# peter-nebe/stair-step-detector

Measured on AMD Instinct MI355X. Metric: point-cloud frames/sec (1024×768 pts) at 1/2/4/8 GPUs; step height/corner max-abs err, higher is better.
Workload: dtype f64; 1 GPU; BASELINE configs[2]: batch of 1024 synthetic 1024x768 frames (3-step staircases, randomised rise/tread/yaw/noise) resident in HBM, streamed through the whole per-frame path; per GPU; width=1024, height=768, input=float3, risers=False, batches_in_flight=3, parallelism=frame-sharded x1, no collective

## Files before the change

include/ssd_testhooks.h:

```cpp
#ifndef SSD_TESTHOOKS_H_
#define SSD_TESTHOOKS_H_

#include "ssd_hip.h"

#ifdef __cplusplus
extern "C" {
#endif

double ssd_test_hypot_host(double a, double b);
int ssd_test_hypot_device(int device, const double *a, const double *b, double *out, int n);
int ssd_test_sort_host(const double *dist, int n, int32_t *perm);
int ssd_test_sort_device(int device, const double *dist, int n, int32_t *perm);
int ssd_test_quad_device(int device, const double quad[8], const double *pts_xy, int n, uint8_t *inside, int *err);
int ssd_test_quad_host(const double quad[8], const double *pts_xy, int n, uint8_t *inside, int *err);
int ssd_test_quad_edges_host(const double quad[8], const double range[6], const double a[9], const double b[3], const float *pts_xyz, int n,
                             float consts[15], int8_t *cls, double *world_xy, uint8_t *in_range_xy, int *err);
int ssd_test_quad_edges_device(int device, const double *quads, int n, const double range_xy[4], float *out);
int ssd_test_best_line_host(const int32_t *pts_xy, int n, int form, int32_t line[3]);
int ssd_test_closing_host(const uint8_t *img, int width, int height, int x0, int x_step, int y_from, int band_rows, uint8_t *closed_out,
                          int32_t *first, int32_t *last, int n_cols);
int ssd_test_grid_boxes_device(int device, const double quad[8], double x_min, double y_min, double box_x, double box_y,
                               const int32_t *boxes, int n, uint8_t *inside, int *usable);
long long ssd_test_frame_state(ssd_handle *h, int frame, void *out, size_t cap, long long layout[8]);
int ssd_test_empty_quadrilateral(ssd_handle *h, int frame, int surface);
int ssd_test_single_pass(ssd_handle *h, int mode, int sabotage);
int ssd_test_plane_pool(ssd_handle *h, int planes);
int ssd_test_single_pass_stats(ssd_handle *h, int frames, int scan_planes, long long counts[4]);
int ssd_test_single_pass_frame(ssd_handle *h, int frame, uint8_t *plane_of_bin, int info[3]);
int ssd_test_single_pass_sample(ssd_handle *h, int frame, uint32_t *sample);
int ssd_test_predict_table_host(const uint32_t *sample, int n_bins, int min_height, int sabotage, uint8_t *plane_of_bin);
int ssd_test_prexy_host(const double range[6], const double a[9], const double b[3], float out[14]);
int ssd_test_prez_host(const double range[6], const double a[9], const double b[3], double height_interval, int width, int height, float out[16]);
int ssd_test_record_offset(ssd_handle *h, size_t offset_bytes);
unsigned long long ssd_test_record_realloc(ssd_handle *h);
unsigned long long ssd_test_record_realloc_sized(ssd_handle *h, size_t extra_bytes, size_t offset_bytes);
int ssd_test_record_release(void);
int ssd_test_ground_image(ssd_handle *h, int frame, uint8_t *out);
int ssd_test_line_host(const double pq[4], double abc_d[3], int32_t abc_i[3]);
int ssd_test_intersect_host(const double l[3], const double o[3], double xy[2]);

int ssd_test_stream_read(int device, const void *d_ptr, size_t bytes, int reps, void *stream, float *ms_avg);

const char *ssd_testhooks_last_error(void);

#ifdef __cplusplus
}
#endif

#endif
```

stair-step-detector_amd/__init__.py:

```python
import ctypes as C
import math
import os

import numpy as np

_HERE = os.path.dirname(os.path.abspath(__file__))
LIB_PATH = os.environ.get("SSD_HIP_LIB") or os.path.join(_HERE, "lib", "libssd_hip.so")

MAX_BINS = 128
MAX_PLATEAUS = 32
MAX_STEP_IMAGES = 16
MAX_PLANES = 24
POOL_PLANES_PER_FRAME = 10


def plane_pool_size(frames, points_per_frame):
    per = 16 if points_per_frame < 600000 else POOL_PLANES_PER_FRAME
    return max(frames * per + 2 * MAX_PLANES, min(frames, 8) * MAX_PLANES)
MAX_STEPS = MAX_STEP_IMAGES + 1
MAX_SCANS = 128
MAX_EDGE_PTS = 256
LINE_CAP = 4096

ST_THROW, ST_OOB_PIXEL, ST_ASSERT, ST_OVERFLOW = 1, 2, 4, 8
# ... 155 lines not shown
                ("seed", C.c_uint64)]


EXPORTS = [
    "ssd_default_config", "ssd_calibration_from_points", "ssd_calibration_identity", "ssd_calibration_load",
    "ssd_create", "ssd_destroy", "ssd_last_error", "ssd_workspace_bytes",
    "ssd_process_host", "ssd_enqueue", "ssd_fetch", "ssd_enqueue_stages",
    "ssd_set_intrinsics", "ssd_process_depth_host", "ssd_enqueue_depth", "ssd_deproject_host",
    "ssd_fetch_back", "ssd_stream_wait", "ssd_batches_in_flight", "ssd_set_risers", "ssd_set_single_pass", "ssd_fetch_risers", "ssd_set_timing", "ssd_get_stage_times", "ssd_get_stage_times_back", "ssd_get_predict_time_back", "ssd_serialize",
    "ssd_set_debug", "ssd_get_debug", "ssd_get_debug_image",
    "ssd_device_count", "ssd_device_alloc", "ssd_device_free", "ssd_device_upload", "ssd_device_download",
    "ssd_device_sync", "ssd_host_alloc", "ssd_host_free", "ssd_device_info_get", "ssd_bind_thread_to_device",
    "ssd_pipeline_create", "ssd_pipeline_destroy", "ssd_pipeline_submit", "ssd_pipeline_submit_after", "ssd_pipeline_next", "ssd_pipeline_pending", "ssd_pipeline_set_timing", "ssd_pipeline_stage_times",
    "ssd_pipeline_last_error",
    "ssd_enqueue_labels", "ssd_enqueue_depth_labels", "ssd_process_host_labels", "ssd_process_depth_host_labels", "ssd_get_labels_time_back",
    "ssd_set_cameras", "ssd_camera_count", "ssd_enqueue_cameras", "ssd_process_host_cameras",
    "ssd_calibration_from_plane", "ssd_ground_moments_host", "ssd_ground_fit_solve", "ssd_enqueue_ground_fit", "ssd_fetch_ground_fit",
    "ssd_process_host_ground_fit",
    "ssd_enqueue_surface_moments", "ssd_enqueue_depth_surface_moments", "ssd_get_surface_moments_time_back", "ssd_surface_moments_host",
    "ssd_surface_fit_solve", "ssd_process_host_surfaces",
    "ssd_enqueue_cameras_surface_moments", "ssd_process_host_cameras_surfaces", "ssd_camera_drift_fold",
    "ssd_set_riser_moments", "ssd_fetch_riser_moments", "ssd_riser_fit_solve", "ssd_process_host_riser_fits",
    "ssd_process_host_cameras_riser_fits",
    "ssd_surface_gates_from_moments", "ssd_surface_refit_moments_host", "ssd_enqueue_surface_refit", "ssd_fetch_surface_refit",
    "ssd_get_surface_refit_time", "ssd_process_host_surfaces_refit",
    "ssd_enqueue_cameras_surface_refit", "ssd_process_host_cameras_surfaces_refit", "ssd_camera_ground_gates",
]
SOURCE_EXPORTS = [
    "ssd_synth_generate_host", "ssd_synth_generate_device", "ssd_synth_depth_host", "ssd_synth_depth_device",
    "ssd_synth_scene_to_camera", "ssd_source_default_scene", "ssd_source_write_calibration", "ssd_source_last_error",
]
HOOK_EXPORTS = [
    "ssd_test_hypot_host", "ssd_test_hypot_device", "ssd_test_frame_state", "ssd_test_ground_image", "ssd_test_line_host", "ssd_test_intersect_host", "ssd_test_quad_device", "ssd_test_quad_host", "ssd_test_closing_host", "ssd_test_best_line_host", "ssd_test_grid_boxes_device", "ssd_test_sort_host",
    "ssd_test_sort_device", "ssd_test_stream_read", "ssd_test_empty_quadrilateral", "ssd_test_single_pass", "ssd_test_plane_pool", "ssd_test_single_pass_stats", "ssd_test_single_pass_frame", "ssd_test_single_pass_sample", "ssd_test_predict_table_host", "ssd_test_prexy_host", "ssd_test_prez_host", "ssd_test_quad_edges_host", "ssd_test_quad_edges_device", "ssd_test_record_offset", "ssd_test_record_realloc", "ssd_test_record_realloc_sized", "ssd_test_record_release", "ssd_testhooks_last_error",
]
SOURCE_LIB_PATH = os.path.join(os.path.dirname(LIB_PATH), "libssd_source.so")
HOOKS_LIB_PATH = os.path.join(os.path.dirname(LIB_PATH), "libssd_testhooks.so")

_lib = None
_source_lib = None
_hooks_lib = None


def lib():
    global _lib
    if _lib is not None:
        return _lib
    if not os.path.exists(LIB_PATH):
        raise SsdError("%s is missing: build it with `python -c 'import __graft_entry__ as g; g.build()'` "
                       "(or make -C stair-step-detector_amd/csrc); there is no CPU fallback" % LIB_PATH)
    L = C.CDLL(LIB_PATH)
    vp, i32, sz = C.c_void_p, C.c_int, C.c_size_t
    L.ssd_last_error.restype = C.c_char_p
    L.ssd_workspace_bytes.restype = sz
    L.ssd_workspace_bytes.argtypes = [vp]
    L.ssd_default_config.argtypes = [C.POINTER(Config), i32, i32]
    L.ssd_calibration_from_points.argtypes = [C.POINTER(C.c_double), C.POINTER(C.c_double), C.POINTER(Calibration)]
    L.ssd_calibration_identity.argtypes = [C.POINTER(Calibration)]
    L.ssd_calibration_load.argtypes = [C.c_char_p, C.c_char_p, C.POINTER(Calibration), C.POINTER(C.c_int),
                                       C.POINTER(C.c_double), C.POINTER(C.c_double)]
    L.ssd_create.argtypes = [C.POINTER(Config), C.POINTER(Calibration), i32, C.POINTER(vp)]
    L.ssd_destroy.argtypes = [vp]
    L.ssd_process_host.argtypes = [vp, vp, i32, C.POINTER(FrameResult)]
    L.ssd_enqueue.argtypes = [vp, vp, sz, i32, vp]
    L.ssd_enqueue_stages.argtypes = [vp, vp, sz, i32, vp, i32]
    L.ssd_fetch.argtypes = [vp, C.POINTER(FrameResult), i32, vp]
    L.ssd_set_intrinsics.argtypes = [vp, C.POINTER(Intrinsics)]
# ... 100 lines not shown
    _source_lib = L
    return L


def hooks_lib():
    global _hooks_lib
    if _hooks_lib is not None:
        return _hooks_lib
    if not os.path.exists(HOOKS_LIB_PATH):
        raise SsdError("%s is missing: build it with make -C stair-step-detector_amd/csrc" % HOOKS_LIB_PATH)
    lib()
    L = C.CDLL(HOOKS_LIB_PATH)
    vp, i32 = C.c_void_p, C.c_int
    L.ssd_testhooks_last_error.restype = C.c_char_p
    L.ssd_test_hypot_host.restype = C.c_double
    L.ssd_test_hypot_host.argtypes = [C.c_double, C.c_double]
    L.ssd_test_hypot_device.argtypes = [i32, vp, vp, vp, i32]
    L.ssd_test_closing_host.argtypes = [vp, i32, i32, i32, i32, i32, i32, vp, vp, vp, i32]
    L.ssd_test_closing_host.restype = i32
    L.ssd_test_best_line_host.argtypes = [vp, i32, i32, vp]
    L.ssd_test_best_line_host.restype = i32
    L.ssd_test_quad_host.argtypes = [vp, vp, i32, vp, vp]
    L.ssd_test_quad_host.restype = i32
    L.ssd_test_frame_state.argtypes = [vp, i32, vp, C.c_size_t, vp]
    L.ssd_test_frame_state.restype = C.c_longlong
    L.ssd_test_ground_image.argtypes = [vp, i32, vp]
    L.ssd_test_empty_quadrilateral.argtypes = [vp, i32, i32]
    L.ssd_test_single_pass.argtypes = [vp, i32, i32]
    L.ssd_test_plane_pool.argtypes = [vp, i32]
    L.ssd_test_single_pass_stats.argtypes = [vp, i32, i32, vp]
    L.ssd_test_single_pass_frame.argtypes = [vp, i32, vp, vp]
    L.ssd_test_single_pass_sample.argtypes = [vp, i32, vp]
    L.ssd_test_predict_table_host.argtypes = [vp, i32, i32, i32, vp]
    L.ssd_test_prexy_host.argtypes = [vp, vp, vp, vp]
    L.ssd_test_prez_host.argtypes = [vp, vp, vp, C.c_double, i32, i32, vp]
    L.ssd_test_quad_edges_host.argtypes = [vp, vp, vp, vp, vp, i32, vp, vp, vp, vp, vp]
    L.ssd_test_quad_edges_host.restype = i32
    L.ssd_test_quad_edges_device.argtypes = [i32, vp, i32, vp, vp]
    L.ssd_test_quad_edges_device.restype = i32
    L.ssd_test_record_offset.argtypes = [vp, C.c_size_t]
    L.ssd_test_record_realloc.argtypes = [vp]
    L.ssd_test_record_realloc.restype = C.c_ulonglong
    L.ssd_test_record_realloc_sized.argtypes = [vp, C.c_size_t, C.c_size_t]
    L.ssd_test_record_realloc_sized.restype = C.c_ulonglong
    L.ssd_test_line_host.argtypes = [vp, vp, vp]
    L.ssd_test_intersect_host.argtypes = [vp, vp, vp]
    L.ssd_test_sort_host.argtypes = [vp, i32, vp]
    L.ssd_test_sort_device.argtypes = [i32, vp, i32, vp]
    L.ssd_test_quad_device.argtypes = [i32, vp, vp, i32, vp, C.POINTER(C.c_int)]
    L.ssd_test_grid_boxes_device.argtypes = [i32, vp, C.c_double, C.c_double, C.c_double, C.c_double, vp, i32, vp, C.POINTER(C.c_int)]
    L.ssd_test_stream_read.argtypes = [i32, vp, C.c_size_t, i32, vp, C.POINTER(C.c_float)]
    _hooks_lib = L
    return L


def _check(rc, which="hip"):
    if rc < 0:
        msg = {"hip": lambda: lib().ssd_last_error(), "source": lambda: source_lib().ssd_source_last_error(),
               "hooks": lambda: hooks_lib().ssd_testhooks_last_error()}[which]().decode()
        raise SsdError("libssd_%s error %d: %s" % (which, rc, msg))
    return rc


def predict_table_host(sample, n_bins, min_height, sabotage=0):
    a = np.ascontiguousarray(sample, dtype=np.uint32)
    assert a.size == MAX_BINS
    out = np.zeros(MAX_BINS, dtype=np.uint8)
    n = _check(hooks_lib().ssd_test_predict_table_host(a.ctypes.data_as(C.c_void_p), n_bins, min_height, sabotage, out.ctypes.data_as(C.c_void_p)), "hooks")
    return out, n


def device_info(device):
    info = DeviceInfo()
    _check(lib().ssd_device_info_get(device, C.byref(info)))
    return {"pci_bus_id": info.pci_bus_id.decode(), "uuid": info.uuid.decode(), "numa_node": int(info.numa_node),
            "n_local_cpus": int(info.n_local_cpus), "cpu_list": info.cpu_list.decode()}


def bind_thread_to_device(device):
    n = lib().ssd_bind_thread_to_device(device)
    if n < 0:
        _check(n)
    return n


def device_count():
    return lib().ssd_device_count()


def default_config(width, height, max_frames_per_batch=64, max_step_plateaus=MAX_STEP_IMAGES, batches_in_flight=0):
    cfg = Config()
    _check(lib().ssd_default_config(C.byref(cfg), width, height))
    cfg.max_frames_per_batch = max_frames_per_batch
    cfg.max_step_plateaus = max_step_plateaus
    cfg.batches_in_flight = batches_in_flight
    return cfg


def _as_camera(prior, intr=None):
    if isinstance(prior, Camera):
        return prior
    if isinstance(prior, (tuple, list)):
# ... 926 lines not shown
```

stair-step-detector_amd/csrc/ssd_kernels.hip:

```cpp
#ifndef SSD_CAMERAS_TU
#define SSD_ENTRY(bounds, kernel, block) __global__ bounds void kernel
#define SSD_BYVAL(T) T
#else
#define SSD_ENTRY(bounds, kernel, block) __device__ __forceinline__ void block
#define SSD_BYVAL(T) const T &
#undef SSD_PHASE_TIMING
#undef SSD_COUNT
#endif
#include "ssd_device.h"
#include "ssd_moments.h"
#include "ssd_math.h"
#include "ssd_quadtest.h"
#include "ssd_closing.h"
#include "ssd_bestline.h"
#include "ssd_sort.h"

namespace ssd
{

#include "ssd_phase.h"

#ifdef SSD_CHECKED
__device__ __noinline__ void ssd_chk_report(int site, unsigned long long idx, unsigned long long limit)
{
  printf("SSD_CHECK site %d index %llu limit %llu block (%u, %u) thread %u\n", site, idx, limit, blockIdx.x, blockIdx.y, threadIdx.x);
}
__device__ __forceinline__ bool ssd_chk(int site, unsigned long long idx, unsigned long long limit)
{
  if(idx < limit)
    return true;
  ssd_chk_report(site, idx, limit);
  return false;
}
#define SSD_CHK(site, idx, limit) ssd_chk((site), static_cast<unsigned long long>(idx), static_cast<unsigned long long>(limit))
#else
#define SSD_CHK(site, idx, limit) (true)
#endif

#ifdef SSD_COUNT
__device__ unsigned long long ssd_k1_counters[8];
#define SSD_CNT(i, n) do { if(threadIdx.x % 64 == 0) atomicAdd(&ssd_k1_counters[i], static_cast<unsigned long long>(n)); } while(0)
#define SSD_CNT_LANES(i, pred) do { const unsigned long long cnt_m = __ballot(pred); if(threadIdx.x % 64 == 0 && cnt_m) atomicAdd(&ssd_k1_counters[i], static_cast<unsigned long long>(__popcll(cnt_m))); } while(0)
#else
#define SSD_CNT(i, n) do { } while(0)
#define SSD_CNT_LANES(i, pred) do { } while(0)
#endif


// ... 1105 lines not shown
__global__ __launch_bounds__(kThreads, SSD_K1S_WAVES) void k_hist_planes(const float *__restrict__ xyz, size_t strideFloats, PointParams P, PreXY Q, PixelParams X,
                                                   FrameState *__restrict__ st, uint2 *__restrict__ tileMasks,
                                                   unsigned long long *__restrict__ planeImg,
                                                   size_t tileMaskStride, int chunkPoints, DepthSrc D)
{
  __shared__ HistLds L;
  __shared__ SpecLds SL;
#ifdef SSD_K1_ROTATE
  const int chunkIdx = static_cast<int>((blockIdx.y + blockIdx.x * SSD_K1_ROTATE) % gridDim.y);
  const int frameIdx = static_cast<int>(blockIdx.x);
#elif defined(SSD_K1_ORDER)
  const int nF = static_cast<int>(gridDim.x), nC = static_cast<int>(gridDim.y);
  const int lin = static_cast<int>(blockIdx.y) * nF + static_cast<int>(blockIdx.x);
  int frameIdx, chunkIdx;
  if(SSD_K1_ORDER == 2 && (nF & 7) == 0)
  {
    const int xcd = lin & 7, i = lin >> 3;
    frameIdx = xcd + 8 * (i / nC);
    chunkIdx = i % nC;
  }
  else
  {
    frameIdx = lin / nC;
    chunkIdx = lin % nC;
  }
#else
  const int chunkIdx = static_cast<int>(blockIdx.y);
  const int frameIdx = static_cast<int>(blockIdx.x);
#endif
  hist_block<SRC, true, STRIPS, CHECKS>(L, SL, xyz, strideFloats, P, Q, X, st, tileMasks, planeImg, tileMaskStride, chunkPoints, D, frameIdx, chunkIdx);
}
#endif

template<int SRC>
SSD_ENTRY(__launch_bounds__(kThreads), k_predict, predict_block)(const float *__restrict__ xyz, size_t strideFloats, SSD_BYVAL(PointParams) P,
                                                      FrameState *__restrict__ st, SSD_BYVAL(DepthSrc) D, int minHeight, int sabotage, int *__restrict__ fallback, int poolPlanes)
{
  __shared__ unsigned int sh[kMaxBins + 2];
  __shared__ unsigned int shc[kMaxBins * kHistCopies];
  __shared__ int sLast;
  const int frame = blockIdx.x, part = blockIdx.y, nParts = gridDim.y, tid = threadIdx.x;
  const float *base = SRC == kSrcDepth16
    ? reinterpret_cast<const float *>(reinterpret_cast<const unsigned short *>(xyz) + static_cast<size_t>(frame) * strideFloats)
    : xyz + static_cast<size_t>(frame) * strideFloats;
  if(tid < kMaxBins + 2)
    sh[tid] = 0u;
  for(int i = tid; i < kMaxBins * kHistCopies; i += kThreads)
    shc[i] = 0u;
  __syncthreads();
  unsigned int *mine = shc + (tid & (kHistCopies - 1));
#ifndef SSD_K0_RUN
#define SSD_K0_RUN 16
#endif
  constexpr int kRun = SSD_K0_RUN, kLanesPerRun = kRun / kPts;
  const int nRuns = (P.nPoints + kRun - 1) / kRun;
  const int nGroups = (nRuns + kSpecSample - 1) / kSpecSample;
  for(int g = part * (kThreads / kLanesPerRun) + tid / kLanesPerRun; g < nGroups; g += nParts * (kThreads / kLanesPerRun))
  {
    const int run = g * kSpecSample + ((g * 5) & (kSpecSample - 1));
    F3 v[kPts];
    load_points<SRC>(base, run * kRun + kPts * (tid % kLanesPerRun), P.nPoints, v, D);
#pragma unroll
    for(int j = 0; j < kPts; j++)
    {
      double wx, wy, wz;
      if(world_point_flat(P, v[j], wx, wy, wz))
        atomicAdd(mine + height_bin(P, wz) * kHistCopies, 1u);
    }
  }
  __syncthreads();
  FrameState &fs = st[frame];
  if(tid < P.nBins)
  {
    unsigned int c = 0;
#pragma unroll
    for(int k = 0; k < kHistCopies; k++)
      c += shc[tid * kHistCopies + ((k + tid) & (kHistCopies - 1))];
    if(c)
    {
      const unsigned int before = atomicAdd(&fs.predHist[tid], c);
      asm volatile("" :: "v"(before));
    }
  }
  __syncthreads();
#if defined(__HIP_DEVICE_COMPILE__) && !defined(__gfx950__)
#error "k_predict's hand-over between blocks is written for gfx950 (see the comment above)"
#endif
  if(tid == 0)
    sLast = atomicAdd(&fs.predDone, 1u) == static_cast<unsigned int>(nParts - 1) ? 1 : 0;
  __syncthreads();
  if(!sLast)
    return;
  const unsigned int mineCount = tid < P.nBins ? atomicExch(&fs.predHist[tid], 0u) : 0u;
  __syncthreads();
  if(tid < kMaxBins)
  {
    sh[1 + tid] = mineCount;
    fs.predSample[tid] = mineCount;
  }
  if(tid == 0)
// ... 59 lines not shown
      if(base + total > poolPlanes)
        base = -1;
    }
    sBase = base;
  }
  __syncthreads();
  const bool fits = sBase >= 0;
  if(tid < kMaxBins)
  {
    const unsigned long long upTo = tid < 64 ? (2ull << tid) - 1ull : ~0ull;
    const int n = tid < 64 ? __popcll(sStart[0] & upTo) : __popcll(sStart[0]) + __popcll(sStart[1] & ((2ull << (tid - 64)) - 1ull));
    fs.specPlane[tid] = (want && fits) ? static_cast<unsigned char>(n - 1) : static_cast<unsigned char>(0xff);
  }
  if(tid < kMaxPlanes)
  {
    fs.planeYMin[tid] = 0x7fffffff; fs.planeYMax[tid] = -1;
    fs.planeXMin[tid] = 0x7fffffff; fs.planeXMax[tid] = -1;
    fs.planeTotZ[tid] = 0;
    fs.planeOob[tid] = 0u;
    fs.planeUsed[tid] = 0;
  }
  if(tid == 0)
  {
    fs.nPlanes = fits ? total : 0;
    fs.planeBase = fits ? sBase : 0;
    fs.predDone = 0u;
    if(frame == 0)
    {
      fallback[0] = 0;
      fallback[1] = 0;
    }
  }
}


SSD_ENTRY(__launch_bounds__(64), k_peaks, peaks_block)(SSD_BYVAL(Params) P, FrameState *__restrict__ st, int nframes, DebugFrame *__restrict__ dbg, int spec, int *__restrict__ fallback)
{
  __shared__ unsigned char sImgPlane[kMaxStepImages][2];
  __shared__ unsigned int sCovered;
  __shared__ unsigned int hist[kMaxBins + 1];
  __shared__ unsigned char lut[kMaxBins];
  __shared__ int plPeak[kMaxPlateaus], plLo[kMaxPlateaus], plHi[kMaxPlateaus], plEffLo[kMaxPlateaus], plEffHi[kMaxPlateaus], plN[kMaxPlateaus];
  __shared__ int dbgPeaks[kMaxPlateaus];
  __shared__ int sNPl, sNPeaks, sOverflow, sGround, sFirstStep, sNImg;

  const int frame = blockIdx.x, lane = threadIdx.x;
  if(frame >= nframes)
    return;
  FrameState &fs = st[frame];
  const int nb = P.nBins;

  unsigned int total = 0;
  for(int b = lane; b <= kMaxBins; b += 64)
  {
    const unsigned int v = b < nb ? fs.histAcc[b] : 0u;
    hist[b] = v;
    total += v;
    if(b < kMaxBins)
    {
      lut[b] = 0xff;
      fs.hist[b] = v;
      if(b < nb)
        fs.histAcc[b] = 0u;
    }
  }
#pragma unroll
// ... 2686 lines not shown
static inline void with_src(const DepthSrc *depth, bool aligned, F f)
{
  if(depth)
    f(std::integral_constant<int, kSrcDepth16>{}, *depth);
  else if(aligned)
    f(std::integral_constant<int, kSrcF3Aligned>{}, DepthSrc{});
  else
    f(std::integral_constant<int, kSrcF3>{}, DepthSrc{});
}
template<typename F>
static inline void with_bool(bool b, F f)
{
  if(b)
    f(std::true_type{});
  else
    f(std::false_type{});
}
}

#ifndef SSD_CAMERAS_TU
namespace ssd
{



void launch_predict(const float *xyz, size_t strideFloats, const Params &P, FrameState *st, int nframes, const DepthSrc *depth,
                    int *fallback, int poolPlanes, int sabotage, hipStream_t s, const CameraSel *cams)
{
  if(cams)
    return launch_predict_cams(xyz, strideFloats, P, st, nframes, depth, fallback, poolPlanes, sabotage, s, *cams);
  dim3 pgrid(nframes, kPredictParts);
  with_src(depth, aligned16(xyz, strideFloats, P.nPoints), [&](auto src, const DepthSrc &D)
  {
    hipLaunchKernelGGL(k_predict<decltype(src)::value>, pgrid, dim3(kThreads), 0, s, xyz, strideFloats, P.pt, st, D, P.minHeight, sabotage, fallback, poolPlanes);
  });
}
void launch_hist(const float *xyz, size_t strideFloats, const Params &P, FrameState *st, uint2 *tileMasks, size_t tileMaskStride,
                 int nframes, int chunkPoints, const DepthSrc *depth, unsigned long long *planeImg, hipStream_t s, const CameraSel *cams)
{
  if(cams)
    return launch_hist_cams(xyz, strideFloats, P, st, tileMasks, tileMaskStride, nframes, chunkPoints, depth, planeImg, s, *cams);
  dim3 grid(nframes, chunks_for(P.nPoints, chunkPoints));
  const bool strips = planeImg && kTile % P.W != 0;
  with_src(depth, aligned16(xyz, strideFloats, P.nPoints), [&](auto src, const DepthSrc &D)
  {
    with_bool(needs_checks(P), [&](auto checks)
    {
      constexpr int SRC = decltype(src)::value;
      constexpr bool CHECKS = decltype(checks)::value;
      if(planeImg)
        with_bool(strips, [&](auto sorted)
        {
          hipLaunchKernelGGL((k_hist_planes<SRC, decltype(sorted)::value, CHECKS>), grid, dim3(kThreads), 0, s, xyz, strideFloats, P.pt, P.pre, P.px, st, tileMasks, planeImg, tileMaskStride, chunkPoints, D);
        });
      else
        hipLaunchKernelGGL((k_hist<SRC, CHECKS>), grid, dim3(kThreads), 0, s, xyz, strideFloats, P.pt, P.pre, st, tileMasks, tileMaskStride, chunkPoints, D);
    });
  });
}
void launch_peaks(const Params &P, FrameState *st, int nframes, DebugFrame *dbg, int *fallback, hipStream_t s, const CameraSel *cams)
{
  if(cams)
    return launch_peaks_cams(P, st, nframes, dbg, fallback, s, *cams);
  hipLaunchKernelGGL(k_peaks, dim3(nframes), dim3(64), 0, s, P, st, nframes, dbg, fallback ? 1 : 0, fallback);
}
void launch_raster(const float *xyz, size_t strideFloats, const Params &P, FrameState *st, unsigned long long *stepImg,
                   const uint2 *tileMasks, size_t tileMaskStride, int nframes, int chunkPoints, const DepthSrc *depth, const int *fallback, hipStream_t s, const CameraSel *cams)
// ... 123 lines not shown
```

stair-step-detector_amd/csrc/ssd_kernels_cams.hip:

```cpp
#define SSD_CAMERAS_TU
#include "ssd_kernels.hip"

namespace ssd
{

template<int SRC, bool CHECKS>
__global__ __launch_bounds__(kThreads, 6) void k_hist_cams(const float *__restrict__ xyz, size_t strideFloats, const CameraRec *__restrict__ cams,
                                                        const int *__restrict__ camOf, FrameState *__restrict__ st, uint2 *__restrict__ tileMasks,
                                                        size_t tileMaskStride, int chunkPoints)
{
  __shared__ HistLds L;
  NoSpecLds none;
  const CameraRec &C = camera_of(cams, camOf, blockIdx.x);
  const PointParams P = C.P.pt;
  const PreXY Q = C.P.pre;
  const DepthSrc D = C.D;
  hist_block<SRC, false, false, CHECKS>(L, none, xyz, strideFloats, P, Q, PixelParams{}, st, tileMasks, nullptr, tileMaskStride, chunkPoints, D, blockIdx.x, blockIdx.y);
}

template<int SRC, bool STRIPS, bool CHECKS>
__global__ __launch_bounds__(kThreads, SSD_K1S_WAVES) void k_hist_planes_cams(const float *__restrict__ xyz, size_t strideFloats, const CameraRec *__restrict__ cams,
                                                   const int *__restrict__ camOf, FrameState *__restrict__ st, uint2 *__restrict__ tileMasks,
                                                   unsigned long long *__restrict__ planeImg, size_t tileMaskStride, int chunkPoints)
{
  __shared__ HistLds L;
  __shared__ SpecLds SL;
  const CameraRec &C = camera_of(cams, camOf, blockIdx.x);
  const PointParams P = C.P.pt;
  const PreXY Q = C.P.pre;
  const PixelParams X = C.P.px;
  const DepthSrc D = C.D;
  hist_block<SRC, true, STRIPS, CHECKS>(L, SL, xyz, strideFloats, P, Q, X, st, tileMasks, planeImg, tileMaskStride, chunkPoints, D, blockIdx.x, blockIdx.y);
}

template<int SRC>
__global__ __launch_bounds__(kThreads) void k_predict_cams(const float *__restrict__ xyz, size_t strideFloats, const CameraRec *__restrict__ cams,
                                                           const int *__restrict__ camOf, FrameState *__restrict__ st, int sabotage, int *__restrict__ fallback, int poolPlanes)
{
  const CameraRec &C = camera_of(cams, camOf, blockIdx.x);
  const PointParams P = C.P.pt;
  const DepthSrc D = C.D;
  predict_block<SRC>(xyz, strideFloats, P, st, D, C.P.minHeight, sabotage, fallback, poolPlanes);
}

__global__ __launch_bounds__(64) void k_peaks_cams(const CameraRec *__restrict__ cams, const int *__restrict__ camOf, FrameState *__restrict__ st, int nframes,
                                                   DebugFrame *__restrict__ dbg, int spec, int *__restrict__ fallback)
{
  if(static_cast<int>(blockIdx.x) >= nframes)
    return;
  peaks_block(camera_of(cams, camOf, blockIdx.x).P, st, nframes, dbg, spec, fallback);
}

template<int SRC, bool LIST>
__global__ __launch_bounds__(kThreads, LIST ? 5 : SSD_K2_WAVES) void k_raster_cams(const float *__restrict__ xyz, size_t strideFloats, const CameraRec *__restrict__ cams,
                                                        const int *__restrict__ camOf, FrameState *__restrict__ st,
                                                        unsigned long long *__restrict__ stepImg,
                                                        const uint2 *__restrict__ tileMasks, size_t tileMaskStride, int chunkPoints,
                                                        const int *__restrict__ fallback)
{
  __shared__ RasterLds L;
  if constexpr(LIST)
  {
    const int n = fallback[0];
    for(int e = blockIdx.x; e < n; e += gridDim.x)
    {
      const int frame = fallback[kFallbackList + e];
      const CameraRec &C = camera_of(cams, camOf, frame);
      const PointParams P = C.P.pt;
      const PixelParams X = C.P.px;
      const DepthSrc D = C.D;
      raster_block<SRC>(L, xyz, strideFloats, P, X, st, stepImg, tileMasks, tileMaskStride, chunkPoints, D, frame, blockIdx.y);
      __syncthreads();
    }
  }
  else
// ... 85 lines not shown
  const PointParams P = C.P.pt;
  const DepthSrc D = C.D;
  risers_block<SRC>(xyz, strideFloats, P, C.P.riserTol, st, tileMasks, tileMaskStride, chunkPoints, C.P.px.cellCols, D);
}

template<int SRC>
__global__ __launch_bounds__(kThreads) void k_riser_moments_cams(const float *__restrict__ xyz, size_t strideFloats, const CameraRec *__restrict__ cams,
                                                                 const int *__restrict__ camOf, FrameState *__restrict__ st, const uint2 *__restrict__ tileMasks,
                                                                 size_t tileMaskStride, int chunkPoints, ssd_frame_moments *__restrict__ out)
{
  const CameraRec &C = camera_of(cams, camOf, blockIdx.x);
  const PointParams P = C.P.pt;
  const DepthSrc D = C.D;
  riser_moments_block<SRC>(xyz, strideFloats, P, C.P.riserTol, st, tileMasks, tileMaskStride, chunkPoints, C.P.px.cellCols, D, out);
}

__global__ void k_riser_results_cams(const CameraRec *__restrict__ cams, const int *__restrict__ camOf, const FrameState *__restrict__ st,
                                     ssd_frame_risers *__restrict__ out, int nframes)
{
  const int frame = blockIdx.x * blockDim.x + threadIdx.x;
  if(frame >= nframes)
    return;
  riser_results_block(cams[camOf[frame]].P, st, out, nframes);
}



void launch_predict_cams(const float *xyz, size_t strideFloats, const Params &P, FrameState *st, int nframes, const DepthSrc *depth,
                         int *fallback, int poolPlanes, int sabotage, hipStream_t s, const CameraSel &cams)
{
  dim3 pgrid(nframes, kPredictParts);
  with_src(depth, aligned16(xyz, strideFloats, P.nPoints), [&](auto src, const DepthSrc &)
  {
    hipLaunchKernelGGL(k_predict_cams<decltype(src)::value>, pgrid, dim3(kThreads), 0, s, xyz, strideFloats, cams.table, cams.index, st, sabotage, fallback, poolPlanes);
  });
}
void launch_hist_cams(const float *xyz, size_t strideFloats, const Params &P, FrameState *st, uint2 *tileMasks, size_t tileMaskStride,
                      int nframes, int chunkPoints, const DepthSrc *depth, unsigned long long *planeImg, hipStream_t s, const CameraSel &cams)
{
  dim3 grid(nframes, chunks_for(P.nPoints, chunkPoints));
  const bool strips = planeImg && kTile % P.W != 0;
  with_src(depth, aligned16(xyz, strideFloats, P.nPoints), [&](auto src, const DepthSrc &)
  {
    with_bool(cams.checks, [&](auto checks)
    {
      constexpr int SRC = decltype(src)::value;
      constexpr bool CHECKS = decltype(checks)::value;
      if(planeImg)
        with_bool(strips, [&](auto sorted)
        {
          hipLaunchKernelGGL((k_hist_planes_cams<SRC, decltype(sorted)::value, CHECKS>), grid, dim3(kThreads), 0, s, xyz, strideFloats, cams.table, cams.index, st, tileMasks, planeImg, tileMaskStride, chunkPoints);
        });
      else
        hipLaunchKernelGGL((k_hist_cams<SRC, CHECKS>), grid, dim3(kThreads), 0, s, xyz, strideFloats, cams.table, cams.index, st, tileMasks, tileMaskStride, chunkPoints);
    });
  });
}
void launch_peaks_cams(const Params &, FrameState *st, int nframes, DebugFrame *dbg, int *fallback, hipStream_t s, const CameraSel &cams)
{
  hipLaunchKernelGGL(k_peaks_cams, dim3(nframes), dim3(64), 0, s, cams.table, cams.index, st, nframes, dbg, fallback ? 1 : 0, fallback);
}
void launch_raster_cams(const float *xyz, size_t strideFloats, const Params &P, FrameState *st, unsigned long long *stepImg,
                        const uint2 *tileMasks, size_t tileMaskStride, int nframes, int chunkPoints, const DepthSrc *depth, const int *fallback, hipStream_t s,
                        const CameraSel &cams)
{
  dim3 grid(fallback ? (nframes + 3) / 4 : nframes, chunks_for(P.nPoints, chunkPoints));
  with_src(depth, aligned16(xyz, strideFloats, P.nPoints), [&](auto src, const DepthSrc &)
// ... 91 lines not shown
```

stair-step-detector_amd/csrc/ssd_predict.h:

```cpp
#ifndef SSD_PREDICT_H_
#define SSD_PREDICT_H_

#include "ssd_device.h"

namespace ssd
{

__host__ __device__ inline bool predict_candidate(const unsigned int *sample, int nBins, int minHeight, int b)
{
  if(b < (minHeight > 1 ? minHeight : 1) || b >= nBins - 1)
    return false;
  const unsigned int c = sample[b], l = sample[b - 1], r = sample[b + 1];
  return c > l && c >= r && c * static_cast<unsigned int>(kSpecSample) >= 1200u && (l + r) * 2u < 3u * c + 16u;
}

__host__ __device__ inline int predict_table(const unsigned int *sample, int nBins, int minHeight, int sabotage, unsigned char *plane)
{
  unsigned char code[kMaxBins];
  for(int b = 0; b < kMaxBins; b++)
  {
    code[b] = 0;
    plane[b] = 0xff;
  }
  if(sabotage == 2)
    return 0;
  for(int b = 0; b < nBins && b < kMaxBins; b++)
  {
    if(!predict_candidate(sample, nBins, minHeight, b))
      continue;
    int fuller = 0;
    for(int o = 0; o < nBins && o < kMaxBins; o++)
      if(o != b && predict_candidate(sample, nBins, minHeight, o) && (sample[o] > sample[b] || (sample[o] == sample[b] && o < b)))
        fuller++;
    if(fuller >= kMaxPlanes / 3)
      continue;
    const unsigned int l = sample[b - 1], r = sample[b + 1];
    code[b] = static_cast<unsigned char>(1u | (r > 2u * l + 8u ? 0u : 2u) | (l > 2u * r + 8u ? 0u : 4u));
  }
  const int shift = sabotage == 1 ? 3 : 0;
// ... 32 lines not shown
```

stair-step-detector_amd/csrc/ssd_testhooks.hip:

```cpp
#include "ssd_handle.h"
#include "ssd_launch.h"
#include "ssd_predict.h"
#include "ssd_prexy.h"
#include "ssd_math.h"
#include "ssd_quadtest.h"
#include "ssd_closing.h"
#include "ssd_bestline.h"
#include "ssd_sort.h"
#include "../../include/ssd_testhooks.h"

#include <cstddef>
#include <cstring>
#include <string>
#include <vector>

using namespace ssd;

namespace
{

thread_local std::string g_err;

int fail(int code, const std::string &msg)
{
// ... 328 lines not shown
    counts[2] += fs.nPlanes;
  }
  return 1;
}

int ssd_test_single_pass_frame(ssd_handle *h, int frame, uint8_t *plane_of_bin, int info[3])
{
  if(!h || !plane_of_bin || !info || frame < 0 || frame >= h->F)
    return fail(SSD_E_ARG, "ssd_test_single_pass_frame: bad argument");
  HIP_TRY(hipSetDevice(h->device));
  HIP_TRY(hipDeviceSynchronize());
  FrameState fs;
  HIP_TRY(hipMemcpy(&fs, h->lane[h->lastLane].dState + frame, sizeof(fs), hipMemcpyDeviceToHost));
  std::memcpy(plane_of_bin, fs.specPlane, kMaxBins);
  info[0] = fs.nPlanes; info[1] = fs.specOk; info[2] = fs.nStepImages;
  return SSD_OK;
}

int ssd_test_single_pass_sample(ssd_handle *h, int frame, uint32_t *sample)
{
  if(!h || !sample || frame < 0 || frame >= h->F)
    return fail(SSD_E_ARG, "ssd_test_single_pass_sample: bad argument");
  HIP_TRY(hipSetDevice(h->device));
  HIP_TRY(hipDeviceSynchronize());
  HIP_TRY(hipMemcpy(sample, h->lane[h->lastLane].dState[frame].predSample, sizeof(unsigned int) * kMaxBins, hipMemcpyDeviceToHost));
  return SSD_OK;
}

int ssd_test_predict_table_host(const uint32_t *sample, int n_bins, int min_height, int sabotage, uint8_t *plane_of_bin)
{
  if(!sample || !plane_of_bin || n_bins < 2 || n_bins > kMaxBins || sabotage < 0 || sabotage > 2)
    return fail(SSD_E_ARG, "ssd_test_predict_table_host: bad argument");
  return predict_table(sample, n_bins, min_height, sabotage, plane_of_bin);
}

int ssd_test_prexy_host(const double range[6], const double a[9], const double b[3], float out[14])
{
  if(!range || !a || !b || !out)
    return fail(SSD_E_ARG, "ssd_test_prexy_host: null");
  PointParams P{};
  for(int i = 0; i < 9; i++) P.a[i] = a[i];
  for(int i = 0; i < 3; i++) P.b[i] = b[i];
  P.xMin = range[0]; P.xMax = range[1]; P.yMin = range[2]; P.yMax = range[3]; P.zMin = range[4]; P.zMax = range[5];
  const PreXY Q = make_pre_xy(P);
  for(int i = 0; i < 4; i++) { out[2 * i] = Q.c[i][0]; out[2 * i + 1] = Q.c[i][1]; }
  out[8] = Q.lo; out[9] = Q.hi; out[10] = Q.maxInput; out[11] = Q.boxLo; out[12] = Q.boxHi; out[13] = static_cast<float>(Q.checkInput);
  return SSD_OK;
}

int ssd_test_prez_host(const double range[6], const double a[9], const double b[3], double height_interval, int width, int height, float out[16])
{
  if(!range || !a || !b || !out || !(height_interval > 0.0) || width <= 0 || height <= 0)
    return fail(SSD_E_ARG, "ssd_test_prez_host: bad argument");
  PointParams P{};
  for(int i = 0; i < 9; i++) P.a[i] = a[i];
  for(int i = 0; i < 3; i++) P.b[i] = b[i];
  P.xMin = range[0]; P.xMax = range[1]; P.yMin = range[2]; P.yMax = range[3]; P.zMin = range[4]; P.zMax = range[5];
  P.recip = 1.0 / height_interval;
  const PreXY Q = make_pre_xy(P);
  PixelParams X{};
  X.W = width; X.H = height;
  X.xToImage = width / (P.xMax - P.xMin);
  X.yToImage = height / (P.yMax - P.yMin);
  make_pre_pixel(P, Q, X);
  for(int i = 0; i < 4; i++) out[i] = Q.zc[i];
  out[4] = Q.zNegK; out[5] = Q.zH0; out[6] = Q.zTop; out[7] = static_cast<float>(Q.zCheckTop);
// ... 321 lines not shown
```

Before: 377,100 frames/s.

## Sample predict histogram by whole cache lines and use float pre-range test

```diff
diff --git a/include/ssd_testhooks.h b/include/ssd_testhooks.h
--- a/include/ssd_testhooks.h
+++ b/include/ssd_testhooks.h
@@ -29,6 +29,7 @@
 int ssd_test_single_pass_frame(ssd_handle *h, int frame, uint8_t *plane_of_bin, int info[3]);
 int ssd_test_single_pass_sample(ssd_handle *h, int frame, uint32_t *sample);
 int ssd_test_predict_table_host(const uint32_t *sample, int n_bins, int min_height, int sabotage, uint8_t *plane_of_bin);
+int ssd_test_predict_sample_host(unsigned long long base_address, int n_points, int32_t *first, int32_t *count, int cap);
 int ssd_test_prexy_host(const double range[6], const double a[9], const double b[3], float out[14]);
 int ssd_test_prez_host(const double range[6], const double a[9], const double b[3], double height_interval, int width, int height, float out[16]);
 int ssd_test_record_offset(ssd_handle *h, size_t offset_bytes);
diff --git a/stair-step-detector_amd/__init__.py b/stair-step-detector_amd/__init__.py
--- a/stair-step-detector_amd/__init__.py
+++ b/stair-step-detector_amd/__init__.py
@@ -211,7 +211,7 @@
 ]
 HOOK_EXPORTS = [
     "ssd_test_hypot_host", "ssd_test_hypot_device", "ssd_test_frame_state", "ssd_test_ground_image", "ssd_test_line_host", "ssd_test_intersect_host", "ssd_test_quad_device", "ssd_test_quad_host", "ssd_test_closing_host", "ssd_test_best_line_host", "ssd_test_grid_boxes_device", "ssd_test_sort_host",
-    "ssd_test_sort_device", "ssd_test_stream_read", "ssd_test_empty_quadrilateral", "ssd_test_single_pass", "ssd_test_plane_pool", "ssd_test_single_pass_stats", "ssd_test_single_pass_frame", "ssd_test_single_pass_sample", "ssd_test_predict_table_host", "ssd_test_prexy_host", "ssd_test_prez_host", "ssd_test_quad_edges_host", "ssd_test_quad_edges_device", "ssd_test_record_offset", "ssd_test_record_realloc", "ssd_test_record_realloc_sized", "ssd_test_record_release", "ssd_testhooks_last_error",
+    "ssd_test_sort_device", "ssd_test_stream_read", "ssd_test_empty_quadrilateral", "ssd_test_single_pass", "ssd_test_plane_pool", "ssd_test_single_pass_stats", "ssd_test_single_pass_frame", "ssd_test_single_pass_sample", "ssd_test_predict_table_host", "ssd_test_predict_sample_host", "ssd_test_prexy_host", "ssd_test_prez_host", "ssd_test_quad_edges_host", "ssd_test_quad_edges_device", "ssd_test_record_offset", "ssd_test_record_realloc", "ssd_test_record_realloc_sized", "ssd_test_record_release", "ssd_testhooks_last_error",
 ]
 SOURCE_LIB_PATH = os.path.join(os.path.dirname(LIB_PATH), "libssd_source.so")
 HOOKS_LIB_PATH = os.path.join(os.path.dirname(LIB_PATH), "libssd_testhooks.so")
@@ -378,6 +378,7 @@
     L.ssd_test_single_pass_frame.argtypes = [vp, i32, vp, vp]
     L.ssd_test_single_pass_sample.argtypes = [vp, i32, vp]
     L.ssd_test_predict_table_host.argtypes = [vp, i32, i32, i32, vp]
+    L.ssd_test_predict_sample_host.argtypes = [C.c_ulonglong, i32, vp, vp, i32]
     L.ssd_test_prexy_host.argtypes = [vp, vp, vp, vp]
     L.ssd_test_prez_host.argtypes = [vp, vp, vp, C.c_double, i32, i32, vp]
     L.ssd_test_quad_edges_host.argtypes = [vp, vp, vp, vp, vp, i32, vp, vp, vp, vp, vp]
@@ -414,6 +415,14 @@
     out = np.zeros(MAX_BINS, dtype=np.uint8)
     n = _check(hooks_lib().ssd_test_predict_table_host(a.ctypes.data_as(C.c_void_p), n_bins, min_height, sabotage, out.ctypes.data_as(C.c_void_p)), "hooks")
     return out, n
+
+
+def predict_sample_host(base_address, n_points):
+    groups = _check(hooks_lib().ssd_test_predict_sample_host(int(base_address), int(n_points), None, None, 0), "hooks")
+    first, count = np.zeros(groups, dtype=np.int32), np.zeros(groups, dtype=np.int32)
+    _check(hooks_lib().ssd_test_predict_sample_host(int(base_address), int(n_points), first.ctypes.data_as(C.c_void_p),
+                                                    count.ctypes.data_as(C.c_void_p), groups), "hooks")
+    return first, count
 
 
 def device_info(device):
diff --git a/stair-step-detector_amd/csrc/ssd_kernels.hip b/stair-step-detector_amd/csrc/ssd_kernels.hip
--- a/stair-step-detector_amd/csrc/ssd_kernels.hip
+++ b/stair-step-detector_amd/csrc/ssd_kernels.hip
@@ -14,6 +14,7 @@
 #include "ssd_closing.h"
 #include "ssd_bestline.h"
 #include "ssd_sort.h"
+#include "ssd_predict.h"
 
 namespace ssd
 {
@@ -1185,12 +1186,13 @@
 }
 #endif
 
-template<int SRC>
-SSD_ENTRY(__launch_bounds__(kThreads), k_predict, predict_block)(const float *__restrict__ xyz, size_t strideFloats, SSD_BYVAL(PointParams) P,
-                                                      FrameState *__restrict__ st, SSD_BYVAL(DepthSrc) D, int minHeight, int sabotage, int *__restrict__ fallback, int poolPlanes)
+template<int SRC, bool CHECKS>
+__device__ __forceinline__ void predict_block(const float *__restrict__ xyz, size_t strideFloats, const PointParams &P, const PreXY &Q,
+                                              FrameState *__restrict__ st, const DepthSrc &D, int minHeight, int sabotage, int *__restrict__ fallback, int poolPlanes)
 {
   __shared__ unsigned int sh[kMaxBins + 2];
-  __shared__ unsigned int shc[kMaxBins * kHistCopies];
+  alignas(16) __shared__ unsigned int shc[kMaxBins * kHistCopies];
+  __shared__ K1Consts kc;
   __shared__ int sLast;
   const int frame = blockIdx.x, part = blockIdx.y, nParts = gridDim.y, tid = threadIdx.x;
   const float *base = SRC == kSrcDepth16
@@ -1198,27 +1200,74 @@
     : xyz + static_cast<size_t>(frame) * strideFloats;
   if(tid < kMaxBins + 2)
     sh[tid] = 0u;
-  for(int i = tid; i < kMaxBins * kHistCopies; i += kThreads)
-    shc[i] = 0u;
+  for(int i = tid; i < kMaxBins * kHistCopies / 4; i += kThreads)
+    reinterpret_cast<uint4 *>(shc)[i] = make_uint4(0u, 0u, 0u, 0u);
+  if(SRC != kSrcDepth16 && tid == 0)
+    k1_consts_fill(kc, P, nullptr);
   __syncthreads();
   unsigned int *mine = shc + (tid & (kHistCopies - 1));
+  if constexpr(SRC != kSrcDepth16)
+  {
+    constexpr int kLines = 64 / kPredictLinePoints, kDepth = 4;
+    const int lane = tid & 63, wave = __builtin_amdgcn_readfirstlane(tid >> 6);
+    const int slot = lane / kPredictLinePoints, k = lane - slot * kPredictLinePoints;
+    const bool live = slot < kLines;
+    const int step = nParts * (kThreads / 64) * kLines;
+    const int gWave = (part * (kThreads / 64) + wave) * kLines;
+    const unsigned long long addr = reinterpret_cast<unsigned long long>(base);
+    const int nGroups = predict_sample_groups(addr, P.nPoints);
+    const PreLane lc(Q);
+    for(int s = 0; gWave + s * step < nGroups; s += kDepth)
+    {
+      F3 v[kDepth];
+      bool has[kDepth];
+#pragma unroll
+      for(int d = 0; d < kDepth; d++)
+      {
+        const PredictRun r = predict_sample_run(addr, P.nPoints, gWave + slot + (s + d) * step);
+        has[d] = live & (k < r.count);
+        v[d] = *reinterpret_cast<const F3 *>(base + 3 * static_cast<size_t>(min(r.first + k, P.nPoints - 1)));
+      }
+#pragma unroll
+      for(int d = 0; d < kDepth; d++)
+      {
+        const F3 p{ v[d].x, v[d].y, has[d] ? v[d].z : 0.0f };
+        const PreRange r = pre_range<CHECKS, false>(p, Q, lc);
+        unsigned int b = r.b;
+        unsigned long long mIn = r.mInSure;
+        if(r.mSlow != 0ull)
+        {
+          const K1ConstsLds c = k1_consts(kc);
+          const World3 w = world_rows(c, p);
+          mIn |= r.mSlow & __ballot(world_in_range(c, w));
+          b = __builtin_amdgcn_inverse_ballot_w64(r.mSlow) ? static_cast<unsigned int>(world_bin(c, w)) : b;
+        }
+        if(__builtin_amdgcn_inverse_ballot_w64(mIn))
+          if(SSD_CHK(32, b, P.nBins))
+            atomicAdd(mine + b * kHistCopies, 1u);
+      }
+    }
+  }
+  else
+  {
 #ifndef SSD_K0_RUN
 #define SSD_K0_RUN 16
 #endif
-  constexpr int kRun = SSD_K0_RUN, kLanesPerRun = kRun / kPts;
-  const int nRuns = (P.nPoints + kRun - 1) / kRun;
-  const int nGroups = (nRuns + kSpecSample - 1) / kSpecSample;
-  for(int g = part * (kThreads / kLanesPerRun) + tid / kLanesPerRun; g < nGroups; g += nParts * (kThreads / kLanesPerRun))
-  {
-    const int run = g * kSpecSample + ((g * 5) & (kSpecSample - 1));
-    F3 v[kPts];
-    load_points<SRC>(base, run * kRun + kPts * (tid % kLanesPerRun), P.nPoints, v, D);
-#pragma unroll
-    for(int j = 0; j < kPts; j++)
-    {
-      double wx, wy, wz;
-      if(world_point_flat(P, v[j], wx, wy, wz))
-        atomicAdd(mine + height_bin(P, wz) * kHistCopies, 1u);
+    constexpr int kRun = SSD_K0_RUN, kLanesPerRun = kRun / kPts;
+    const int nRuns = (P.nPoints + kRun - 1) / kRun;
+    const int nGroups = (nRuns + kSpecSample - 1) / kSpecSample;
+    for(int g = part * (kThreads / kLanesPerRun) + tid / kLanesPerRun; g < nGroups; g += nParts * (kThreads / kLanesPerRun))
+    {
+      const int run = g * kSpecSample + ((g * 5) & (kSpecSample - 1));
+      F3 v[kPts];
+      load_points<SRC>(base, run * kRun + kPts * (tid % kLanesPerRun), P.nPoints, v, D);
+#pragma unroll
+      for(int j = 0; j < kPts; j++)
+      {
+        double wx, wy, wz;
+        if(world_point_flat(P, v[j], wx, wy, wz))
+          atomicAdd(mine + height_bin(P, wz) * kHistCopies, 1u);
+      }
     }
   }
   __syncthreads();
@@ -1344,6 +1393,21 @@
     }
   }
 }
+
+#ifndef SSD_CAMERAS_TU
+template<int SRC>
+__global__ __launch_bounds__(kThreads) void k_predict(const float *__restrict__ xyz, size_t strideFloats, PointParams P, PreXY Q, FrameState *__restrict__ st, DepthSrc D,
+                                                      int minHeight, int sabotage, int *__restrict__ fallback, int poolPlanes)
+{
+  predict_block<SRC, false>(xyz, strideFloats, P, Q, st, D, minHeight, sabotage, fallback, poolPlanes);
+}
+template<int SRC>
+__global__ __launch_bounds__(kThreads) void k_predict_checks(const float *__restrict__ xyz, size_t strideFloats, PointParams P, PreXY Q, FrameState *__restrict__ st, DepthSrc D,
+                                                             int minHeight, int sabotage, int *__restrict__ fallback, int poolPlanes)
+{
+  predict_block<SRC, true>(xyz, strideFloats, P, Q, st, D, minHeight, sabotage, fallback, poolPlanes);
+}
+#endif
 
 
 SSD_ENTRY(__launch_bounds__(64), k_peaks, peaks_block)(SSD_BYVAL(Params) P, FrameState *__restrict__ st, int nframes, DebugFrame *__restrict__ dbg, int spec, int *__restrict__ fallback)
@@ -4096,7 +4160,14 @@
   dim3 pgrid(nframes, kPredictParts);
   with_src(depth, aligned16(xyz, strideFloats, P.nPoints), [&](auto src, const DepthSrc &D)
   {
-    hipLaunchKernelGGL(k_predict<decltype(src)::value>, pgrid, dim3(kThreads), 0, s, xyz, strideFloats, P.pt, st, D, P.minHeight, sabotage, fallback, poolPlanes);
+    constexpr int SRC = decltype(src)::value;
+    if constexpr(SRC != kSrcDepth16)
+      if(needs_checks(P))
+      {
+        hipLaunchKernelGGL(k_predict_checks<SRC>, pgrid, dim3(kThreads), 0, s, xyz, strideFloats, P.pt, P.pre, st, D, P.minHeight, sabotage, fallback, poolPlanes);
+        return;
+      }
+    hipLaunchKernelGGL(k_predict<SRC>, pgrid, dim3(kThreads), 0, s, xyz, strideFloats, P.pt, P.pre, st, D, P.minHeight, sabotage, fallback, poolPlanes);
   });
 }
 void launch_hist(const float *xyz, size_t strideFloats, const Params &P, FrameState *st, uint2 *tileMasks, size_t tileMaskStride,
diff --git a/stair-step-detector_amd/csrc/ssd_kernels_cams.hip b/stair-step-detector_amd/csrc/ssd_kernels_cams.hip
--- a/stair-step-detector_amd/csrc/ssd_kernels_cams.hip
+++ b/stair-step-detector_amd/csrc/ssd_kernels_cams.hip
@@ -33,14 +33,15 @@
   hist_block<SRC, true, STRIPS, CHECKS>(L, SL, xyz, strideFloats, P, Q, X, st, tileMasks, planeImg, tileMaskStride, chunkPoints, D, blockIdx.x, blockIdx.y);
 }
 
-template<int SRC>
+template<int SRC, bool CHECKS>
 __global__ __launch_bounds__(kThreads) void k_predict_cams(const float *__restrict__ xyz, size_t strideFloats, const CameraRec *__restrict__ cams,
                                                            const int *__restrict__ camOf, FrameState *__restrict__ st, int sabotage, int *__restrict__ fallback, int poolPlanes)
 {
   const CameraRec &C = camera_of(cams, camOf, blockIdx.x);
   const PointParams P = C.P.pt;
-  const DepthSrc D = C.D;
-  predict_block<SRC>(xyz, strideFloats, P, st, D, C.P.minHeight, sabotage, fallback, poolPlanes);
+  const PreXY Q = C.P.pre;
+  const DepthSrc D = C.D;
+  predict_block<SRC, CHECKS>(xyz, strideFloats, P, Q, st, D, C.P.minHeight, sabotage, fallback, poolPlanes);
 }
 
 __global__ __launch_bounds__(64) void k_peaks_cams(const CameraRec *__restrict__ cams, const int *__restrict__ camOf, FrameState *__restrict__ st, int nframes,
@@ -192,7 +193,14 @@
   dim3 pgrid(nframes, kPredictParts);
   with_src(depth, aligned16(xyz, strideFloats, P.nPoints), [&](auto src, const DepthSrc &)
   {
-    hipLaunchKernelGGL(k_predict_cams<decltype(src)::value>, pgrid, dim3(kThreads), 0, s, xyz, strideFloats, cams.table, cams.index, st, sabotage, fallback, poolPlanes);
+    constexpr int SRC = decltype(src)::value;
+    if constexpr(SRC == kSrcDepth16)
+      hipLaunchKernelGGL((k_predict_cams<SRC, false>), pgrid, dim3(kThreads), 0, s, xyz, strideFloats, cams.table, cams.index, st, sabotage, fallback, poolPlanes);
+    else
+      with_bool(cams.checks, [&](auto checks)
+      {
+        hipLaunchKernelGGL((k_predict_cams<SRC, decltype(checks)::value>), pgrid, dim3(kThreads), 0, s, xyz, strideFloats, cams.table, cams.index, st, sabotage, fallback, poolPlanes);
+      });
   });
 }
 void launch_hist_cams(const float *xyz, size_t strideFloats, const Params &P, FrameState *st, uint2 *tileMasks, size_t tileMaskStride,
diff --git a/stair-step-detector_amd/csrc/ssd_predict.h b/stair-step-detector_amd/csrc/ssd_predict.h
--- a/stair-step-detector_amd/csrc/ssd_predict.h
+++ b/stair-step-detector_amd/csrc/ssd_predict.h
@@ -5,6 +5,41 @@
 
 namespace ssd
 {
+
+constexpr int kPredictLineBytes = 128, kPredictPointBytes = 12;
+constexpr int kPredictLinePoints = (kPredictLineBytes - 8) / kPredictPointBytes;
+constexpr int kPredictGroupLines = kSpecSample * kPredictLinePoints * kPredictPointBytes / kPredictLineBytes;
+static_assert(kPredictGroupLines * kPredictLineBytes == kSpecSample * kPredictLinePoints * kPredictPointBytes,
+              "a group of lines must hold kSpecSample times the points of one line");
+
+struct PredictRun { int first, count; };
+
+__host__ __device__ inline unsigned int predict_sample_offset(unsigned int g)
+{
+  return (((g * 0x02D346BEu) >> 16) * static_cast<unsigned int>(kPredictGroupLines)) >> 16;
+}
+__host__ __device__ inline int predict_sample_groups(unsigned long long base, int nPoints)
+{
+  const unsigned int a7 = static_cast<unsigned int>(base) & static_cast<unsigned int>(kPredictLineBytes - 1);
+  const unsigned int lines = (a7 + static_cast<unsigned int>(nPoints) * kPredictPointBytes + kPredictLineBytes - 1) / kPredictLineBytes;
+  return static_cast<int>((lines + kPredictGroupLines - 1) / kPredictGroupLines);
+}
+__host__ __device__ inline PredictRun predict_sample_run(unsigned long long base, int nPoints, int group)
+{
+  const unsigned int a7 = static_cast<unsigned int>(base) & static_cast<unsigned int>(kPredictLineBytes - 1);
+  const unsigned int g = static_cast<unsigned int>(group);
+  const unsigned int line = g * kPredictGroupLines + predict_sample_offset(g);
+  const unsigned int hi = (line + 1u) * kPredictLineBytes - a7;
+  const unsigned int lo = hi - kPredictLineBytes;
+  const unsigned int first = hi <= static_cast<unsigned int>(kPredictLineBytes) ? 0u : (lo + kPredictPointBytes - 1) / kPredictPointBytes;
+  const unsigned int whole = hi / kPredictPointBytes;
+  const unsigned int end = whole < static_cast<unsigned int>(nPoints) ? whole : static_cast<unsigned int>(nPoints);
+  PredictRun r;
+  r.first = static_cast<int>(first);
+  r.count = end > first ? static_cast<int>(end - first) : 0;
+  return r;
+}
+
 
 __host__ __device__ inline bool predict_candidate(const unsigned int *sample, int nBins, int minHeight, int b)
 {
diff --git a/stair-step-detector_amd/csrc/ssd_testhooks.hip b/stair-step-detector_amd/csrc/ssd_testhooks.hip
--- a/stair-step-detector_amd/csrc/ssd_testhooks.hip
+++ b/stair-step-detector_amd/csrc/ssd_testhooks.hip
@@ -384,6 +384,20 @@
   if(!sample || !plane_of_bin || n_bins < 2 || n_bins > kMaxBins || sabotage < 0 || sabotage > 2)
     return fail(SSD_E_ARG, "ssd_test_predict_table_host: bad argument");
   return predict_table(sample, n_bins, min_height, sabotage, plane_of_bin);
+}
+
+int ssd_test_predict_sample_host(unsigned long long base_address, int n_points, int32_t *first, int32_t *count, int cap)
+{
+  if(n_points < 1 || n_points > (1 << 26) || cap < 0 || (cap > 0 && (!first || !count)))
+    return fail(SSD_E_ARG, "ssd_test_predict_sample_host: bad argument");
+  const int groups = predict_sample_groups(base_address, n_points);
+  for(int g = 0; g < groups && g < cap; g++)
+  {
+    const PredictRun r = predict_sample_run(base_address, n_points, g);
+    first[g] = r.first;
+    count[g] = r.count;
+  }
+  return groups;
 }
 
 int ssd_test_prexy_host(const double range[6], const double a[9], const double b[3], float out[14])
```

Result: faster. 386,100 frames/s, median of 6 (+2.4%).
